# wolearyc/ramannoodle

Hardware: AMD Instinct MI355X
Metric: structures/sec (GNN polarizability eval) (higher is better)
Workload: dtype f32

## Files before the change

### ramannoodle_amd/csrc/kernels_c2_pairs.hip

```cpp
#include "fused_common.hpp"

namespace rn {

struct C2PairArgs {
  const float *node;
  float *out;
  int64_t M;
  int N, NP;
  const int *pair_a, *pair_b;
  Dims d;
  PassW<float> w;
};

namespace {
constexpr int C2P_THREADS = 256;
}

__global__ __launch_bounds__(C2P_THREADS, 2) void c2_pairs_kernel(C2PairArgs a) {
  __shared__ __attribute__((aligned(16))) float s_bias[2 * FP], s_g1[2 * FP], s_b1[2 * FP], s_g2[FP], s_b2[FP];
  const int tid = threadIdx.x, lane = tid & 63, wave = tid >> 6;
  const int l15 = lane & 15, quad = lane >> 4;
  const float sc2 = a.w.mfma_scale_c[4];
  for (int c = tid; c < 2 * FP; c += C2P_THREADS) {
    s_bias[c] = a.w.c2_bias_c[c] * sc2;
    s_g1[c] = a.w.c2_norm_1.g[c];
    s_b1[c] = a.w.c2_norm_1.b[c];
    if (c < FP) {
      s_g2[c] = a.w.c2_norm_2.g[c];
      s_b2[c] = a.w.c2_norm_2.b[c];
    }
  }
  WaveB<true> bW[4];
#pragma unroll
  for (int p = 0; p < 4; ++p) bW[p].load(a.w.c2_WT_c, 2 * FP, 32 * p, l15, quad, sc2);
  __syncthreads();

  const float inv2n = 1.0f / (float)(2 * a.d.Fe), invn = 1.0f / (float)a.d.Fe;
  const float eps_c2 = 1e-5f * sc2 * sc2;
  const int64_t ntiles = (a.M + 15) / 16, stride = (int64_t)gridDim.x * (C2P_THREADS / 64);

  f32x4 xb[4], xa[4];
  auto fetch = [&](int64_t tile) {
    int64_t row = tile * 16 + l15;
    if (row >= a.M) row = a.M - 1;
    const int64_t s = row / a.NP;
    const int p = (int)(row - s * a.NP);
    const float *nb = a.node + (s * a.N + a.pair_b[p]) * FP + 16 * quad, *na = a.node + (s * a.N + a.pair_a[p]) * FP + 16 * quad;
#pragma unroll
    for (int j = 0; j < 4; ++j) {
      xb[j] = *reinterpret_cast<const f32x4 *>(nb + 4 * j);
      xa[j] = *reinterpret_cast<const f32x4 *>(na + 4 * j);
    }
  };
  int64_t tile = (int64_t)blockIdx.x * (C2P_THREADS / 64) + wave;
  if (tile < ntiles) fetch(tile);
  for (; tile < ntiles; tile += stride) {
    float af[KS];
#pragma unroll
    for (int j = 0; j < 4; ++j) {
      const f32x4 pr = xb[j] * xa[j];
#pragma unroll
      for (int i = 0; i < 4; ++i) af[4 * j + i] = pr[i];
    }
    f16x8 ah[2], al[2];
    split_f16x8(af, ah[0], al[0]);
    split_f16x8(af + 8, ah[1], al[1]);
    if (tile + stride < ntiles) fetch(tile + stride);

    const int lq = launder(lane >> 4);
    f32x4 acc[4][2];
#pragma unroll
    for (int p = 0; p < 4; ++p) {
#pragma unroll
      for (int t = 0; t < 2; ++t) acc[p][t] = *reinterpret_cast<const f32x4 *>(s_bias + 32 * p + 16 * t + 4 * lq);
      bW[p].product_split(ah, al, acc[p]);
    }
    float q = 0.f;
#pragma unroll
    for (int p = 0; p < 4; ++p)
#pragma unroll
      for (int t = 0; t < 2; ++t)
#pragma unroll
        for (int i = 0; i < 4; ++i) q = fmaf(acc[p][t][i], acc[p][t][i], q);
    q = sum_xor32(sum_xor16(q));
    const float rstd2 = fast_rsq(q * inv2n + eps_c2);
    float gv[2][2][4], sum = 0.f;
#pragma unroll
    for (int p = 0; p < 2; ++p)
#pragma unroll
      for (int t = 0; t < 2; ++t) {
        const int c = 32 * p + 16 * t + 4 * lq;
        const Vec4<float> gf = load4<float>(s_g1 + c), bf = load4<float>(s_b1 + c);
        const Vec4<float> gc = load4<float>(s_g1 + FP + c), bc = load4<float>(s_b1 + FP + c);
#pragma unroll
        for (int i = 0; i < 4; ++i) {
          gv[p][t][i] = gate(acc[p][t][i] * rstd2 * gf.v[i] + bf.v[i], acc[p + 2][t][i] * rstd2 * gc.v[i] + bc.v[i]);
          sum += gv[p][t][i];
        }
      }
    const float mean = sum_xor32(sum_xor16(sum)) * invn;
    float qq = 0.f;
#pragma unroll
    for (int p = 0; p < 2; ++p)
#pragma unroll
      for (int t = 0; t < 2; ++t)
#pragma unroll
        for (int i = 0; i < 4; ++i) {
          const int c = 32 * p + 16 * t + 4 * lq + i;
          gv[p][t][i] = c < a.d.Fe ? gv[p][t][i] - mean : 0.f;
          qq = fmaf(gv[p][t][i], gv[p][t][i], qq);
        }
    const float rstd = fast_rsq(sum_xor32(sum_xor16(qq)) * invn + 1e-5f);
    const int64_t row = tile * 16 + l15 < a.M ? tile * 16 + l15 : a.M - 1;
    {
#pragma unroll
      for (int p = 0; p < 2; ++p)
#pragma unroll
        for (int t = 0; t < 2; ++t) {
          const int c = 32 * p + 16 * t + 4 * lq;
          const Vec4<float> g2 = load4<float>(s_g2 + c), b2 = load4<float>(s_b2 + c);
          f32x4 y;
#pragma unroll
          for (int i = 0; i < 4; ++i) y[i] = gv[p][t][i] * rstd * g2.v[i] + b2.v[i];
          *reinterpret_cast<f32x4 *>(a.out + row * FP + c) = y;
        }
    }
  }
}

void launch_c2_pairs(const float *node, float *out, int S, const Graph &g, Dims d, const PassW<float> &w, hipStream_t st) {
  const int64_t M = (int64_t)S * g.NP;
  if (M == 0) return;
  C2PairArgs a{node, out, M, g.N, g.NP, g.pair_a, g.pair_b, d, w};
  static int cus = 0;
  if (cus == 0) {
    int dev = 0;
    hipDeviceProp_t prop;
    if (hipGetDevice(&dev) == hipSuccess && hipGetDeviceProperties(&prop, dev) == hipSuccess) cus = prop.multiProcessorCount;
    if (cus <= 0) cus = 256;
  }
  const int64_t ntiles = (M + 15) / 16, per_wg = C2P_THREADS / 64;
  const int64_t grid = std::min<int64_t>((ntiles + per_wg - 1) / per_wg, (int64_t)2 * cus);
  c2_pairs_kernel<<<(unsigned)grid, C2P_THREADS, 0, st>>>(a);
}

}
```

### ramannoodle_amd/csrc/kernels_fused.hip

```cpp
#include "fused_common.hpp"

namespace rn {


#ifndef RN_NODE_REGRING
#define RN_NODE_REGRING 2
#endif
#ifndef RN_NODE_PROBE
#define RN_NODE_PROBE 0
#endif
template <bool PAD, bool F16, bool ZM = false >
__global__ __launch_bounds__(256, 4) void node_block_fused_kernel(NodeFusedArgs a) {
  extern __shared__ __attribute__((aligned(16))) unsigned char smem_raw[];
  const Graph &g = a.g;
  const NodeFusedLds L = node_fused_lds(g.nt_max_in_rows, g.nt_max_nodes);
  float *bufP = reinterpret_cast<float *>(smem_raw + L.bufP);
  float *atile = reinterpret_cast<float *>(smem_raw + L.atile);
  float *gated = reinterpret_cast<float *>(smem_raw + L.gated);
  float *nj = reinterpret_cast<float *>(smem_raw + L.nj);
  float *lnp = reinterpret_cast<float *>(smem_raw + L.lnp);
  float *s_c1g = lnp, *s_c1b = lnp + 2 * FP, *s_fg = lnp + 4 * FP, *s_fb = lnp + 5 * FP;
  int *d_edge = reinterpret_cast<int *>(smem_raw + L.ints), *d_bl = d_edge + g.nt_max_in_rows;

  const int tid = threadIdx.x, lane = tid & 63;
  const int wave = __builtin_amdgcn_readfirstlane(tid >> 6);
  const int l15 = lane & 15, quad = lane >> 4;
  const int colbase = wave * 32;
  int logical = blockIdx.x;
  if ((gridDim.x & 7) == 0) logical = (blockIdx.x & 7) * (gridDim.x >> 3) + (blockIdx.x >> 3);
  const int tile = logical % g.nt_num;
  const int sg = logical / g.nt_num, nsg = gridDim.x / g.nt_num;
  const int j0 = g.nt_begin[tile], j1 = g.nt_begin[tile + 1];
  const int di0 = g.in_ptr[j0], dcount = g.in_ptr[j1] - di0;
  const int nrounds = (dcount + NG - 1) / NG;

  for (int c = tid; c < 2 * FP; c += 256) {
    s_c1g[c] = a.w.c1_norm.g[c];
    s_c1b[c] = a.w.c1_norm.b[c];
    if (c < FP) {
      s_fg[c] = a.w.final_norm.g[c];
      s_fb[c] = a.w.final_norm.b[c];
    }
  }
  for (int i = tid; i < dcount; i += 256) {
    const int e = g.in_edge[di0 + i];
    d_edge[i] = e;
    d_bl[i] = g.edge_b[e] - j0;
  }
  WaveB<F16> bW;
  const float s1 = F16 ? (ZM ? a.w.mfma_scale_c[6] : a.w.mfma_scale[0]) : 1.0f, inv1 = F16 ? (ZM ? a.w.mfma_scale_c[7] : a.w.mfma_scale[1]) : 1.0f;
  bW.load(ZM ? a.w.c1_WeT_c : a.w.c1_WeT, 2 * FP, colbase, l15, quad, s1);

  const int grp = tid / LG, q4 = tid % LG, c0 = 4 * q4;
  const int nvalid = min(max(a.d.Fn - c0, 0), 4);
  const float inv2n = 1.0f / (float)(2 * a.d.Fn), invn = 1.0f / (float)a.d.Fn;
  __syncthreads();
  const LnParams<float> pf{load4<float>(s_c1g + c0), load4<float>(s_c1b + c0)};
  const LnParams<float> pc{load4<float>(s_c1g + FP + c0), load4<float>(s_c1b + FP + c0)};

  [[maybe_unused]] auto prefetch_round = [&](int s, int r) {
    const int row = 4 * wave + quad;
    const int i = min(r * NG + row, dcount - 1);
    const int piece = (l15 ^ row) & 15;
    dma16(a.edge + ((int64_t)s * g.E + d_edge[i]) * FP + 4 * piece, atile + wave * 256);
  };
  [[maybe_unused]] auto split_landed_tiles = [&]() {
    if constexpr (F16) {
      float *slot = atile + wave * 256 + lane * 4;
      *reinterpret_cast<float4 *>(slot) = split_slot(*reinterpret_cast<const float4 *>(slot));
    }
  };
#if RN_NODE_REGRING
  constexpr int RING = RN_NODE_REGRING;
  float4 ring[RING];
  int fs = sg, fr = 0;
  auto fetch_next = [&]() {
    float4 v = make_float4(0.f, 0.f, 0.f, 0.f);
    if (fs < a.S) {
      const int row = 4 * wave + quad;
      const int i = min(fr * NG + row, dcount - 1);
      const int piece = (l15 ^ row) & 15;
      v = *reinterpret_cast<const float4 *>(a.edge + ((int64_t)fs * g.E + d_edge[i]) * FP + 4 * piece);
      if (++fr == nrounds) {
        fr = 0;
        fs += nsg;
      }
    }
    return v;
  };
  auto publish_next = [&]() {
    float4 v = ring[0];
    if constexpr (F16) v = split_slot(v);
    *reinterpret_cast<float4 *>(atile + tid * 4) = v;
#pragma unroll
    for (int j = 0; j + 1 < RING; ++j) ring[j] = ring[j + 1];
    ring[RING - 1] = fetch_next();
  };
  if (dcount > 0) {
#pragma unroll
    for (int j = 0; j < RING; ++j) ring[j] = fetch_next();
    if (sg < a.S) publish_next();
  }
#else
  if (sg < a.S && dcount > 0) prefetch_round(sg, 0);
#endif

  for (int s = sg; s < a.S; s += nsg) {
    const int64_t nrow0 = (int64_t)s * g.N;
    for (int i = tid; i < ((RN_NODE_PROBE & 8) ? 0 : (j1 - j0) * (2 * FP / 4)); i += 256) {
      const int n = i / (2 * FP / 4), c = (i % (2 * FP / 4)) * 4;
      store4(nj + (size_t)n * 2 * FP + c, load4<float>(a.npc1 + (nrow0 + j0 + n) * (2 * FP) + c));
    }
#if !RN_NODE_REGRING
    dma_wait();
    if (s == sg) split_landed_tiles();
#endif
    __syncthreads();
    for (int r = 0; r < nrounds; ++r) {
      if (!(RN_NODE_PROBE & 1)) {
        f32x4 acc[2] = {{0.f, 0.f, 0.f, 0.f}, {0.f, 0.f, 0.f, 0.f}};
        if constexpr (F16) {
          f16x8 ah[2], al[2];
          load_split_a(atile, l15, quad, ah, al);
          bW.product_split(ah, al, acc);
        } else {
          float af[KS];
#pragma unroll
          for (int j = 0; j < 4; ++j) {
            const float4 v = *reinterpret_cast<const float4 *>(atile + l15 * FP + (((4 * quad + j) ^ l15) & 15) * 4);
            af[4 * j] = v.x; af[4 * j + 1] = v.y; af[4 * j + 2] = v.z; af[4 * j + 3] = v.w;
          }
          bW.product(af, acc);
        }
#pragma unroll
        for (int t = 0; t < 2; ++t) *reinterpret_cast<f32x4 *>(bufP + l15 * LDQ + colbase + 16 * t + 4 * quad) = acc[t];
      }
      if (!(RN_NODE_PROBE & 32))
      __syncthreads();
#if RN_NODE_REGRING
      if (r + 1 < nrounds || s + nsg < a.S) publish_next();
#else
      if (r + 1 < nrounds) prefetch_round(s, r + 1);
      else if (s + nsg < a.S) prefetch_round(s + nsg, 0);
#endif
#if RN_NODE_PRIO
      __builtin_amdgcn_s_setprio(0);
#endif
      const int i = r * NG + grp;
      if (i < dcount && !(RN_NODE_PROBE & 2)) {
        const float *njr = nj + (size_t)d_bl[i] * 2 * FP + c0;
        Vec4<float> xf = load4<float>(bufP + grp * LDQ + c0), xc = load4<float>(bufP + grp * LDQ + FP + c0);
        const Vec4<float> af = load4<float>(njr), ac = load4<float>(njr + FP);
#pragma unroll
        for (int k = 0; k < 4; ++k) {
          xf.v[k] = fmaf(xf.v[k], inv1, af.v[k]);
          xc.v[k] = fmaf(xc.v[k], inv1, ac.v[k]);
        }
        if constexpr (ZM) store4(gated + (size_t)i * LDG + c0, ln_gate_zero_mean<LG>(xf, xc, pf, pc, inv2n));
        else store4(gated + (size_t)i * LDG + c0, ln_gate<LG, PAD>(xf, xc, pf, pc, inv2n, nvalid));
      }
#if RN_NODE_PRIO
      __builtin_amdgcn_s_setprio(RN_NODE_PRIO);
#endif
#if !RN_NODE_REGRING
      dma_wait();
      if (r + 1 < nrounds || s + nsg < a.S) split_landed_tiles();
#endif
      if (!(RN_NODE_PROBE & 16) || r + 1 == nrounds)
      __syncthreads();
    }
    for (int n = grp; n < ((RN_NODE_PROBE & 4) ? 0 : j1 - j0); n += NG) {
      const int i0 = g.in_ptr[j0 + n] - di0, i1 = g.in_ptr[j0 + n + 1] - di0;
      Vec4<float> acc{{0.f, 0.f, 0.f, 0.f}};
      for (int i = i0; i < i1; ++i) {
        const Vec4<float> v = load4<float>(gated + (size_t)i * LDG + c0);
#pragma unroll
        for (int k = 0; k < 4; ++k) acc.v[k] += v.v[k];
      }
      const LnParams<float> pn{load4<float>(s_fg + c0), load4<float>(s_fb + c0)};
      const Vec4<float> ln = ln_row<LG, PAD>(acc, pn, invn, nvalid);
      const Vec4<float> old = load4<float>(a.node_in + (nrow0 + j0 + n) * FP + c0);
      Vec4<float> out;
#pragma unroll
      for (int k = 0; k < 4; ++k) out.v[k] = fast_tanh(old.v[k] + ln.v[k]);
      store4(a.node_out + (nrow0 + j0 + n) * FP + c0, out);
    }
  }
}

size_t node_fused_lds_bytes(const Graph &g) { return node_fused_lds(g.nt_max_in_rows, g.nt_max_nodes).total; }
size_t node_fused_lds_bytes(int tile_in_rows, int tile_nodes) { return node_fused_lds(tile_in_rows, tile_nodes).total; }

void launch_node_fused(const float *edge, const float *node_in, const float *npc1, float *node_out, int S,
                       const Graph &g, Dims d, const PassW<float> &w, bool f16, bool centred, hipStream_t st) {
  if (S == 0 || g.N == 0) return;
  NodeFusedArgs a{edge, node_in, npc1, node_out, S, g, d, w};
  const bool pad = d.Fn != d.FnP;
  const size_t lds = node_fused_lds_bytes(g);
  auto kern = f16 ? (centred ? (pad ? &node_block_fused_kernel<true, true, true> : &node_block_fused_kernel<false, true, true>)
                             : (pad ? &node_block_fused_kernel<true, true> : &node_block_fused_kernel<false, true>))
                  : (pad ? &node_block_fused_kernel<true, false> : &node_block_fused_kernel<false, false>);
  if (lds > 48 * 1024)
    (void)hipFuncSetAttribute(reinterpret_cast<const void *>(kern), hipFuncAttributeMaxDynamicSharedMemorySize,
                              (int)lds);
  static int cus = 0;
  if (cus == 0) {
    int dev = 0;
    hipDeviceProp_t prop;
    if (hipGetDevice(&dev) == hipSuccess && hipGetDeviceProperties(&prop, dev) == hipSuccess)
      cus = prop.multiProcessorCount;
    if (cus <= 0) cus = 256;
  }
  int per_cu = 0;
  if (hipOccupancyMaxActiveBlocksPerMultiprocessor(&per_cu, kern, 256, lds) != hipSuccess || per_cu < 1) per_cu = 1;
  per_cu = std::min(per_cu, 4);
  int nsg = per_cu * cus / g.nt_num;
  nsg = nsg < 1 ? 1 : (nsg > S ? S : nsg);
  kern<<<(unsigned)nsg * (unsigned)g.nt_num, 256, lds, st>>>(a);
}

struct ReadoutFusedArgs {
  const float *edge;
  float *pol;
  int64_t M;
  ReadoutW<float> w;
  int pol_stride;
};

template <bool F16, bool PRE = false, int NW = (F16 ? 8 : 4)>
__global__ __launch_bounds__(64 * NW, 2) void readout_fused_kernel(ReadoutFusedArgs a, int tiles_per_wave) {
  constexpr int LDW = FP + 4;
  constexpr int LDH = FP + 8;
  constexpr int kW64 = F16 ? 2 * FP * LDH * 2 : FP * LDW * 4, kW16 = F16 ? 2 * 16 * LDH * 2 : 16 * LDW * 4;
  extern __shared__ __attribute__((aligned(16))) unsigned char ro_smem[];
  unsigned char *w0_raw = ro_smem, *w3_raw = w0_raw + kW64, *w5_raw = w3_raw + kW64;
  float *slab_all = reinterpret_cast<float *>(w5_raw + kW16);
  float *s_scale0 = slab_all + NW * 16 * LDW, *s_shift0 = s_scale0 + FP, *s_b3 = s_shift0 + FP, *s_b5 = s_b3 + FP;
  const int tid = threadIdx.x, lane = tid & 63, wave = tid >> 6;
  const int l15 = lane & 15, quad = lane >> 4;
  auto put = [&](unsigned char *raw, int rows, int n, int k, float v) {
    if constexpr (F16) {
      _Float16 *h = reinterpret_cast<_Float16 *>(raw), *l = h + rows * LDH;
      const _Float16 hi = (_Float16)v;
      h[n * LDH + k] = hi;
      l[n * LDH + k] = (_Float16)(v - (float)hi);
    } else {
      reinterpret_cast<float *>(raw)[n * LDW + k] = v;
    }
  };
  const float ps0 = F16 ? a.w.mfma_scale[0] : 1.0f, inv0 = F16 ? a.w.mfma_scale[1] : 1.0f;
  const float ps3 = F16 ? a.w.mfma_scale[2] : 1.0f, inv3 = F16 ? a.w.mfma_scale[3] : 1.0f;
  const float ps5 = F16 ? a.w.mfma_scale[4] : 1.0f, inv5 = F16 ? a.w.mfma_scale[5] : 1.0f;
  for (int i = tid; i < FP * FP; i += 64 * NW) {
    const int k = i / FP, n = i % FP;
    put(w0_raw, FP, n, k, ps0 * a.w.W0T[i]);
    put(w3_raw, FP, n, k, ps3 * a.w.W3T[i]);
  }
  for (int i = tid; i < FP * 16; i += 64 * NW) {
    const int k = i / 16, n = i % 16;
    put(w5_raw, 16, n, k, ps5 * a.w.W5T[k * 32 + n]);
  }
  if (tid < FP) {
    s_scale0[tid] = a.w.scale0[tid] * inv0;
    s_shift0[tid] = a.w.shift0[tid];
    s_b3[tid] = a.w.b3[tid];
    if (tid < 16) s_b5[tid] = a.w.b5[tid];
  }
  __syncthreads();
  float *slab = slab_all + wave * 16 * LDW;
  const int64_t num_tiles = (a.M + 15) / 16;
  const int64_t first = ((int64_t)blockIdx.x * NW + wave) * tiles_per_wave;

  f16x8 ah[2], al[2];
  auto operand = [&](const float (&af)[KS]) {
    if constexpr (F16) {
      split_f16x8(af, ah[0], al[0]);
      split_f16x8(af + 8, ah[1], al[1]);
    }
  };
  auto operand_pairs = [&](const float (&af)[KS]) {
    union { float f[4]; f16x8 h; } u[4];
#pragma unroll
    for (int j = 0; j < 4; ++j)
#pragma unroll
      for (int i = 0; i < 4; ++i) u[j].f[i] = af[4 * j + i];
    ah[0] = u[0].h; al[0] = u[1].h; ah[1] = u[2].h; al[1] = u[3].h;
  };
  auto product = [&](const float (&af)[KS], const unsigned char *raw, int rows, int nt, f32x4 &acc) {
    acc = f32x4{0.f, 0.f, 0.f, 0.f};
    if constexpr (F16) {
      const _Float16 *h = reinterpret_cast<const _Float16 *>(raw) + (nt * 16 + l15) * LDH + quad * KS;
      const _Float16 *l = h + rows * LDH;
#pragma unroll
      for (int s = 0; s < 2; ++s)
        acc = mfma_split3(ah[s], al[s], *reinterpret_cast<const f16x8 *>(h + 8 * s),
                          *reinterpret_cast<const f16x8 *>(l + 8 * s), acc);
    } else {
      const float *wp = reinterpret_cast<const float *>(raw) + (nt * 16 + l15) * LDW + quad * KS;
#pragma unroll
      for (int j = 0; j < 4; ++j) {
        const float4 b = *reinterpret_cast<const float4 *>(wp + 4 * j);
        acc = __builtin_amdgcn_mfma_f32_16x16x4f32(af[4 * j], b.x, acc, 0, 0, 0);
        acc = __builtin_amdgcn_mfma_f32_16x16x4f32(af[4 * j + 1], b.y, acc, 0, 0, 0);
        acc = __builtin_amdgcn_mfma_f32_16x16x4f32(af[4 * j + 2], b.z, acc, 0, 0, 0);
        acc = __builtin_amdgcn_mfma_f32_16x16x4f32(af[4 * j + 3], b.w, acc, 0, 0, 0);
      }
    }
  };
  auto load_slab = [&](float (&af)[KS]) {
#pragma unroll
    for (int j = 0; j < 4; ++j) {
      const float4 v = *reinterpret_cast<const float4 *>(slab + l15 * LDW + quad * KS + 4 * j);
      af[4 * j] = v.x; af[4 * j + 1] = v.y; af[4 * j + 2] = v.z; af[4 * j + 3] = v.w;
    }
  };

  float nxt[KS];
  auto fetch = [&](int64_t tile) {
    int64_t row = tile * 16 + l15;
    if (row >= a.M) row = a.M - 1;
    const float *p = a.edge + row * FP + quad * KS;
#pragma unroll
    for (int j = 0; j < 4; ++j) {
      const float4 v = *reinterpret_cast<const float4 *>(p + 4 * j);
      nxt[4 * j] = v.x; nxt[4 * j + 1] = v.y; nxt[4 * j + 2] = v.z; nxt[4 * j + 3] = v.w;
    }
  };
  if (first < num_tiles) fetch(first);
  for (int it = 0; it < tiles_per_wave; ++it) {
    const int64_t tile = first + it;
    if (tile >= num_tiles) break;
    float af[KS];
#pragma unroll
    for (int k = 0; k < KS; ++k) af[k] = nxt[k];
    if (it + 1 < tiles_per_wave && tile + 1 < num_tiles) fetch(tile + 1);
    f32x4 acc;
    if constexpr (PRE) operand_pairs(af);
    else operand(af);
#pragma unroll
    for (int nt = 0; nt < 4; ++nt) {
      product(af, w0_raw, FP, nt, acc);
      const int col = nt * 16 + l15;
#pragma unroll
      for (int rr = 0; rr < 4; ++rr)
        slab[(4 * quad + rr) * LDW + col] = ssp_fast(acc[rr] * s_scale0[col] + s_shift0[col]);
    }
    load_slab(af);
    operand(af);
#pragma unroll
    for (int nt = 0; nt < 4; ++nt) {
      product(af, w3_raw, FP, nt, acc);
      const int col = nt * 16 + l15;
#pragma unroll
      for (int rr = 0; rr < 4; ++rr) slab[(4 * quad + rr) * LDW + col] = ssp_fast(fmaf(acc[rr], inv3, s_b3[col]));
    }
    load_slab(af);
    operand(af);
    product(af, w5_raw, 16, 0, acc);
#pragma unroll
    for (int rr = 0; rr < 4; ++rr) {
      const int64_t row = tile * 16 + 4 * quad + rr;
      if (row < a.M) a.pol[row * a.pol_stride + l15] = fmaf(acc[rr], inv5, s_b5[l15]);
    }
  }
}

void launch_readout_fused(const float *edge, int64_t M, const ReadoutW<float> &w, float *pol, bool f16,
                          hipStream_t st, bool pair_rows, int pol_stride) {
  if (M == 0) return;
  ReadoutFusedArgs a{edge, pol, M, w, pol_stride};
  const int64_t tiles = (M + 15) / 16;
  const int tpw = 8;
  auto launch = [&](auto kern, int nw, bool f16w) {
    constexpr int LDW = FP + 4, LDH = FP + 8;
    const size_t lds = (f16w ? (size_t)2 * (2 * FP * LDH * 2) + 2 * 16 * LDH * 2 : (size_t)2 * FP * LDW * 4 + 16 * LDW * 4) +
                       (size_t)nw * 16 * LDW * 4 + (3 * FP + 16) * 4;
    if (lds > 48 * 1024)
      (void)hipFuncSetAttribute(reinterpret_cast<const void *>(kern), hipFuncAttributeMaxDynamicSharedMemorySize, (int)lds);
    const unsigned blocks = (unsigned)((tiles + (int64_t)nw * tpw - 1) / ((int64_t)nw * tpw));
    kern<<<blocks, 64 * nw, lds, st>>>(a, tpw);
  };
  if (f16 && pair_rows) launch(&readout_fused_kernel<true, true>, 8, true);
  else if (f16) launch(&readout_fused_kernel<true>, 8, true);
  else launch(&readout_fused_kernel<false>, 4, false);
}

size_t edge_fused_lds_bytes(const Graph &g) {
  return fused_lds(g.max_tile_out_rows, g.max_tile_in_rows, g.max_tile_nodes).total;
}
size_t edge_fused_lds_bytes(int rows, int in_rows, int nodes) { return fused_lds(rows, in_rows, nodes).total; }

bool edge_fused_supported(const Graph &g, Dims d) {
  return d.FnP == 64 && d.FeP == 64 && g.E > 0 && edge_fused_lds_bytes(g) <= kFusedLdsBudget;
}

}
```

Before: 64480.

## Fold log2e into norm params, pack f32x2 math, and transpose readout MFMA outputs

In the c2 pairs kernel, the gate's exp scaling is folded into the norm-1 gamma and beta so a custom exp2-based gate with clamping can be used. Elementwise math moves to packed f32x2 FMAs, and a PAD template skips the padding mask when Fe equals FP. Per-tile 64-bit divides for pair index lookup are replaced by an incremental (s,p) stepper with byte-offset addressing. In the readout kernel, the MFMA operands are swapped so each lane writes four contiguous columns as one vector LDS store, and softplus is rewritten with exp2/log using prescaled biases. The changes trade exact exp/log paths for approximate hardware intrinsics and add more complex index bookkeeping.

```diff
diff --git a/ramannoodle_amd/csrc/kernels_c2_pairs.hip b/ramannoodle_amd/csrc/kernels_c2_pairs.hip
--- a/ramannoodle_amd/csrc/kernels_c2_pairs.hip
+++ b/ramannoodle_amd/csrc/kernels_c2_pairs.hip
@@ -6,7 +6,8 @@
   const float *node;
   float *out;
   int64_t M;
-  int N, NP;
+  int S, N, NP;
+  int step_s, step_p;
   const int *pair_a, *pair_b;
   Dims d;
   PassW<float> w;
@@ -14,17 +15,33 @@
 
 namespace {
 constexpr int C2P_THREADS = 256;
-}
-
+constexpr float kC2Clamp = 15.0f * 2.0f * kLog2e;
+
+__device__ __forceinline__ f32x2 gate_exp2(f32x2 yf, f32x2 yc) {
+  const f32x2 one2 = {1.0f, 1.0f};
+  const f32x2 e1 = {fast_exp2(yf.x), fast_exp2(yf.y)};
+  const f32x2 e2 = {fast_exp2(__builtin_amdgcn_fmed3f(yc.x, -kC2Clamp, kC2Clamp)),
+                    fast_exp2(__builtin_amdgcn_fmed3f(yc.y, -kC2Clamp, kC2Clamp))};
+  const f32x2 t = e2 + one2;
+  const f32x2 den = __builtin_elementwise_fma(e1, t, t);
+  const f32x2 rd = {fast_rcp(den.x), fast_rcp(den.y)};
+  return (e2 - one2) * rd;
+}
+__device__ __forceinline__ f32x2 lo2(const f32x4 &v) { return f32x2{v[0], v[1]}; }
+__device__ __forceinline__ f32x2 hi2(const f32x4 &v) { return f32x2{v[2], v[3]}; }
+}
+
+template <bool PAD>
 __global__ __launch_bounds__(C2P_THREADS, 2) void c2_pairs_kernel(C2PairArgs a) {
   __shared__ __attribute__((aligned(16))) float s_bias[2 * FP], s_g1[2 * FP], s_b1[2 * FP], s_g2[FP], s_b2[FP];
-  const int tid = threadIdx.x, lane = tid & 63, wave = tid >> 6;
+  const int tid = threadIdx.x, lane = tid & 63, wave = __builtin_amdgcn_readfirstlane(tid >> 6);
   const int l15 = lane & 15, quad = lane >> 4;
   const float sc2 = a.w.mfma_scale_c[4];
   for (int c = tid; c < 2 * FP; c += C2P_THREADS) {
+    const float k = c < FP ? -kLog2e : 2.0f * kLog2e;
     s_bias[c] = a.w.c2_bias_c[c] * sc2;
-    s_g1[c] = a.w.c2_norm_1.g[c];
-    s_b1[c] = a.w.c2_norm_1.b[c];
+    s_g1[c] = k * a.w.c2_norm_1.g[c];
+    s_b1[c] = k * a.w.c2_norm_1.b[c];
     if (c < FP) {
       s_g2[c] = a.w.c2_norm_2.g[c];
       s_b2[c] = a.w.c2_norm_2.b[c];
@@ -38,22 +55,55 @@
   const float inv2n = 1.0f / (float)(2 * a.d.Fe), invn = 1.0f / (float)a.d.Fe;
   const float eps_c2 = 1e-5f * sc2 * sc2;
   const int64_t ntiles = (a.M + 15) / 16, stride = (int64_t)gridDim.x * (C2P_THREADS / 64);
-
+  int64_t tile = (int64_t)blockIdx.x * (C2P_THREADS / 64) + wave;
+  if (tile >= ntiles) return;
+
+  constexpr unsigned ROWB = FP * sizeof(float);
+  const uint64_t frame_b = (uint64_t)a.N * ROWB, step_fb = (uint64_t)a.step_s * frame_b;
+  const uint64_t last_fb = (uint64_t)(a.S - 1) * frame_b;
+  int s, p;
+  {
+    const int64_t row = tile * 16 + l15;
+    s = (int)(row / a.NP);
+    p = (int)(row - (int64_t)s * a.NP);
+  }
+  uint64_t fb = (uint64_t)s * frame_b;
+
+  int ia, ib;
+  const char *frame;
+  auto step = [&]() {
+    const bool past = s >= a.S;
+    const int pp = past ? a.NP - 1 : p;
+    frame = reinterpret_cast<const char *>(a.node) + (past ? last_fb : fb);
+    ib = a.pair_b[pp];
+    ia = a.pair_a[pp];
+    p += a.step_p;
+    s += a.step_s;
+    fb += step_fb;
+    if (p >= a.NP) {
+      p -= a.NP;
+      ++s;
+      fb += frame_b;
+    }
+  };
   f32x4 xb[4], xa[4];
-  auto fetch = [&](int64_t tile) {
-    int64_t row = tile * 16 + l15;
-    if (row >= a.M) row = a.M - 1;
-    const int64_t s = row / a.NP;
-    const int p = (int)(row - s * a.NP);
-    const float *nb = a.node + (s * a.N + a.pair_b[p]) * FP + 16 * quad, *na = a.node + (s * a.N + a.pair_a[p]) * FP + 16 * quad;
+  auto fetch = [&](const char *fr, int ja, int jb, int q) {
+    const float *nb = reinterpret_cast<const float *>(fr + ((unsigned)jb * ROWB + 16 * (unsigned)sizeof(float) * q));
+    const float *na = reinterpret_cast<const float *>(fr + ((unsigned)ja * ROWB + 16 * (unsigned)sizeof(float) * q));
 #pragma unroll
     for (int j = 0; j < 4; ++j) {
       xb[j] = *reinterpret_cast<const f32x4 *>(nb + 4 * j);
       xa[j] = *reinterpret_cast<const f32x4 *>(na + 4 * j);
     }
   };
-  int64_t tile = (int64_t)blockIdx.x * (C2P_THREADS / 64) + wave;
-  if (tile < ntiles) fetch(tile);
+  {
+    step();
+    const char *fr0 = frame;
+    const int ia0 = ia, ib0 = ib;
+    step();
+    asm volatile("" ::: "memory");
+    fetch(fr0, ia0, ib0, quad);
+  }
   for (; tile < ntiles; tile += stride) {
     float af[KS];
 #pragma unroll
@@ -65,73 +115,96 @@
     f16x8 ah[2], al[2];
     split_f16x8(af, ah[0], al[0]);
     split_f16x8(af + 8, ah[1], al[1]);
-    if (tile + stride < ntiles) fetch(tile + stride);
-
-    const int lq = launder(lane >> 4);
+    const int ln = launder(lane), lq = ln >> 4;
+    if (tile + stride < ntiles) fetch(frame, ia, ib, lq);
+    step();
+
     f32x4 acc[4][2];
 #pragma unroll
-    for (int p = 0; p < 4; ++p) {
-#pragma unroll
-      for (int t = 0; t < 2; ++t) acc[p][t] = *reinterpret_cast<const f32x4 *>(s_bias + 32 * p + 16 * t + 4 * lq);
-      bW[p].product_split(ah, al, acc[p]);
-    }
-    float q = 0.f;
-#pragma unroll
-    for (int p = 0; p < 4; ++p)
+    for (int pp = 0; pp < 4; ++pp) {
+#pragma unroll
+      for (int t = 0; t < 2; ++t) acc[pp][t] = *reinterpret_cast<const f32x4 *>(s_bias + 32 * pp + 16 * t + 4 * lq);
+    }
+#pragma unroll
+    for (int pp = 0; pp < 4; ++pp) bW[pp].product_split(ah, al, acc[pp]);
+    f32x4 gf[2][2], bf[2][2], gc[2][2], bc[2][2];
+#pragma unroll
+    for (int pp = 0; pp < 2; ++pp)
+#pragma unroll
+      for (int t = 0; t < 2; ++t) {
+        const int c = 32 * pp + 16 * t + 4 * lq;
+        gf[pp][t] = *reinterpret_cast<const f32x4 *>(s_g1 + c);
+        bf[pp][t] = *reinterpret_cast<const f32x4 *>(s_b1 + c);
+        gc[pp][t] = *reinterpret_cast<const f32x4 *>(s_g1 + FP + c);
+        bc[pp][t] = *reinterpret_cast<const f32x4 *>(s_b1 + FP + c);
+      }
+    f32x2 q2[2] = {{0.f, 0.f}, {0.f, 0.f}};
+#pragma unroll
+    for (int pp = 0; pp < 4; ++pp)
+#pragma unroll
+      for (int t = 0; t < 2; ++t) {
+        q2[0] = __builtin_elementwise_fma(lo2(acc[pp][t]), lo2(acc[pp][t]), q2[0]);
+        q2[1] = __builtin_elementwise_fma(hi2(acc[pp][t]), hi2(acc[pp][t]), q2[1]);
+      }
+    const f32x2 qs = q2[0] + q2[1];
+    const float q = sum_xor32(sum_xor16(qs.x + qs.y));
+    const float rstd2 = fast_rsq(q * inv2n + eps_c2);
+    const f32x2 r2 = {rstd2, rstd2};
+    f32x2 gv[2][2][2], sum2 = {0.f, 0.f};
+#pragma unroll
+    for (int pp = 0; pp < 2; ++pp)
+#pragma unroll
+      for (int t = 0; t < 2; ++t) {
+        gv[pp][t][0] = gate_exp2(__builtin_elementwise_fma(lo2(acc[pp][t]) * r2, lo2(gf[pp][t]), lo2(bf[pp][t])),
+                                 __builtin_elementwise_fma(lo2(acc[pp + 2][t]) * r2, lo2(gc[pp][t]), lo2(bc[pp][t])));
+        gv[pp][t][1] = gate_exp2(__builtin_elementwise_fma(hi2(acc[pp][t]) * r2, hi2(gf[pp][t]), hi2(bf[pp][t])),
+                                 __builtin_elementwise_fma(hi2(acc[pp + 2][t]) * r2, hi2(gc[pp][t]), hi2(bc[pp][t])));
+        sum2 += gv[pp][t][0] + gv[pp][t][1];
+      }
+    const float mean = sum_xor32(sum_xor16(sum2.x + sum2.y)) * invn;
+    const f32x2 m2 = {mean, mean};
+    f32x2 qq2 = {0.f, 0.f};
+#pragma unroll
+    for (int pp = 0; pp < 2; ++pp)
 #pragma unroll
       for (int t = 0; t < 2; ++t)
 #pragma unroll
-        for (int i = 0; i < 4; ++i) q = fmaf(acc[p][t][i], acc[p][t][i], q);
-    q = sum_xor32(sum_xor16(q));
-    const float rstd2 = fast_rsq(q * inv2n + eps_c2);
-    float gv[2][2][4], sum = 0.f;
-#pragma unroll
-    for (int p = 0; p < 2; ++p)
-#pragma unroll
-      for (int t = 0; t < 2; ++t) {
-        const int c = 32 * p + 16 * t + 4 * lq;
-        const Vec4<float> gf = load4<float>(s_g1 + c), bf = load4<float>(s_b1 + c);
-        const Vec4<float> gc = load4<float>(s_g1 + FP + c), bc = load4<float>(s_b1 + FP + c);
-#pragma unroll
-        for (int i = 0; i < 4; ++i) {
-          gv[p][t][i] = gate(acc[p][t][i] * rstd2 * gf.v[i] + bf.v[i], acc[p + 2][t][i] * rstd2 * gc.v[i] + bc.v[i]);
-          sum += gv[p][t][i];
+        for (int h = 0; h < 2; ++h) {
+          gv[pp][t][h] -= m2;
+          if constexpr (PAD) {
+            const int c = 32 * pp + 16 * t + 4 * lq + 2 * h;
+            if (c >= a.d.Fe) gv[pp][t][h].x = 0.f;
+            if (c + 1 >= a.d.Fe) gv[pp][t][h].y = 0.f;
+          }
+          qq2 = __builtin_elementwise_fma(gv[pp][t][h], gv[pp][t][h], qq2);
         }
-      }
-    const float mean = sum_xor32(sum_xor16(sum)) * invn;
-    float qq = 0.f;
-#pragma unroll
-    for (int p = 0; p < 2; ++p)
-#pragma unroll
-      for (int t = 0; t < 2; ++t)
-#pragma unroll
-        for (int i = 0; i < 4; ++i) {
-          const int c = 32 * p + 16 * t + 4 * lq + i;
-          gv[p][t][i] = c < a.d.Fe ? gv[p][t][i] - mean : 0.f;
-          qq = fmaf(gv[p][t][i], gv[p][t][i], qq);
-        }
-    const float rstd = fast_rsq(sum_xor32(sum_xor16(qq)) * invn + 1e-5f);
-    const int64_t row = tile * 16 + l15 < a.M ? tile * 16 + l15 : a.M - 1;
-    {
-#pragma unroll
-      for (int p = 0; p < 2; ++p)
-#pragma unroll
-        for (int t = 0; t < 2; ++t) {
-          const int c = 32 * p + 16 * t + 4 * lq;
-          const Vec4<float> g2 = load4<float>(s_g2 + c), b2 = load4<float>(s_b2 + c);
-          f32x4 y;
-#pragma unroll
-          for (int i = 0; i < 4; ++i) y[i] = gv[p][t][i] * rstd * g2.v[i] + b2.v[i];
-          *reinterpret_cast<f32x4 *>(a.out + row * FP + c) = y;
-        }
-    }
+    f32x4 g2[2][2], b2[2][2];
+#pragma unroll
+    for (int pp = 0; pp < 2; ++pp)
+#pragma unroll
+      for (int t = 0; t < 2; ++t) {
+        const int c = 32 * pp + 16 * t + 4 * lq;
+        g2[pp][t] = *reinterpret_cast<const f32x4 *>(s_g2 + c);
+        b2[pp][t] = *reinterpret_cast<const f32x4 *>(s_b2 + c);
+      }
+    const float rstd = fast_rsq(sum_xor32(sum_xor16(qq2.x + qq2.y)) * invn + 1e-5f);
+    const f32x2 rs2 = {rstd, rstd};
+    const unsigned last = (unsigned)std::min<int64_t>(a.M - tile * 16, 16) - 1u, lrow = (unsigned)(ln & 15);
+    char *orow = reinterpret_cast<char *>(a.out) + tile * (16 * ROWB) + ((lrow < last ? lrow : last) * ROWB + 4 * (unsigned)sizeof(float) * lq);
+#pragma unroll
+    for (int pp = 0; pp < 2; ++pp)
+#pragma unroll
+      for (int t = 0; t < 2; ++t) {
+        const f32x2 y0 = __builtin_elementwise_fma(gv[pp][t][0] * rs2, lo2(g2[pp][t]), lo2(b2[pp][t]));
+        const f32x2 y1 = __builtin_elementwise_fma(gv[pp][t][1] * rs2, hi2(g2[pp][t]), hi2(b2[pp][t]));
+        *reinterpret_cast<f32x4 *>(orow + (32 * pp + 16 * t) * sizeof(float)) = f32x4{y0.x, y0.y, y1.x, y1.y};
+      }
   }
 }
 
 void launch_c2_pairs(const float *node, float *out, int S, const Graph &g, Dims d, const PassW<float> &w, hipStream_t st) {
   const int64_t M = (int64_t)S * g.NP;
   if (M == 0) return;
-  C2PairArgs a{node, out, M, g.N, g.NP, g.pair_a, g.pair_b, d, w};
   static int cus = 0;
   if (cus == 0) {
     int dev = 0;
@@ -141,7 +214,10 @@
   }
   const int64_t ntiles = (M + 15) / 16, per_wg = C2P_THREADS / 64;
   const int64_t grid = std::min<int64_t>((ntiles + per_wg - 1) / per_wg, (int64_t)2 * cus);
-  c2_pairs_kernel<<<(unsigned)grid, C2P_THREADS, 0, st>>>(a);
-}
-
-}
+  const int64_t step_rows = grid * per_wg * 16;
+  C2PairArgs a{node, out, M, S, g.N, g.NP, (int)(step_rows / g.NP), (int)(step_rows % g.NP), g.pair_a, g.pair_b, d, w};
+  if (d.Fe < FP) c2_pairs_kernel<true><<<(unsigned)grid, C2P_THREADS, 0, st>>>(a);
+  else c2_pairs_kernel<false><<<(unsigned)grid, C2P_THREADS, 0, st>>>(a);
+}
+
+}
diff --git a/ramannoodle_amd/csrc/kernels_fused.hip b/ramannoodle_amd/csrc/kernels_fused.hip
--- a/ramannoodle_amd/csrc/kernels_fused.hip
+++ b/ramannoodle_amd/csrc/kernels_fused.hip
@@ -227,6 +227,13 @@
   int pol_stride;
 };
 
+namespace {
+__device__ __forceinline__ float ssp_exp2(float y) {
+  const float t = __builtin_amdgcn_exp2f(-fabsf(y));
+  return fmaf(0.6931471805599453f, fmaxf(y, 0.0f) + __builtin_amdgcn_logf(1.0f + t), -0.6931471805599453f);
+}
+}
+
 template <bool F16, bool PRE = false, int NW = (F16 ? 8 : 4)>
 __global__ __launch_bounds__(64 * NW, 2) void readout_fused_kernel(ReadoutFusedArgs a, int tiles_per_wave) {
   constexpr int LDW = FP + 4;
@@ -251,6 +258,7 @@
   const float ps0 = F16 ? a.w.mfma_scale[0] : 1.0f, inv0 = F16 ? a.w.mfma_scale[1] : 1.0f;
   const float ps3 = F16 ? a.w.mfma_scale[2] : 1.0f, inv3 = F16 ? a.w.mfma_scale[3] : 1.0f;
   const float ps5 = F16 ? a.w.mfma_scale[4] : 1.0f, inv5 = F16 ? a.w.mfma_scale[5] : 1.0f;
+  const float inv3l = inv3 * kLog2e;
   for (int i = tid; i < FP * FP; i += 64 * NW) {
     const int k = i / FP, n = i % FP;
     put(w0_raw, FP, n, k, ps0 * a.w.W0T[i]);
@@ -261,9 +269,9 @@
     put(w5_raw, 16, n, k, ps5 * a.w.W5T[k * 32 + n]);
   }
   if (tid < FP) {
-    s_scale0[tid] = a.w.scale0[tid] * inv0;
-    s_shift0[tid] = a.w.shift0[tid];
-    s_b3[tid] = a.w.b3[tid];
+    s_scale0[tid] = a.w.scale0[tid] * inv0 * kLog2e;
+    s_shift0[tid] = a.w.shift0[tid] * kLog2e;
+    s_b3[tid] = a.w.b3[tid] * kLog2e;
     if (tid < 16) s_b5[tid] = a.w.b5[tid];
   }
   __syncthreads();
@@ -307,11 +315,33 @@
       }
     }
   };
+  auto product_t = [&](const float (&af)[KS], const unsigned char *raw, int rows, int nt, f32x4 &acc) {
+    acc = f32x4{0.f, 0.f, 0.f, 0.f};
+    if constexpr (F16) {
+      const _Float16 *h = reinterpret_cast<const _Float16 *>(raw) + (nt * 16 + l15) * LDH + quad * KS;
+      const _Float16 *l = h + rows * LDH;
+#pragma unroll
+      for (int s = 0; s < 2; ++s)
+        acc = mfma_split3(*reinterpret_cast<const f16x8 *>(h + 8 * s), *reinterpret_cast<const f16x8 *>(l + 8 * s), ah[s],
+                          al[s], acc);
+    } else {
+      const float *wp = reinterpret_cast<const float *>(raw) + (nt * 16 + l15) * LDW + quad * KS;
+#pragma unroll
+      for (int j = 0; j < 4; ++j) {
+        const float4 b = *reinterpret_cast<const float4 *>(wp + 4 * j);
+        acc = __builtin_amdgcn_mfma_f32_16x16x4f32(b.x, af[4 * j], acc, 0, 0, 0);
+        acc = __builtin_amdgcn_mfma_f32_16x16x4f32(b.y, af[4 * j + 1], acc, 0, 0, 0);
+        acc = __builtin_amdgcn_mfma_f32_16x16x4f32(b.z, af[4 * j + 2], acc, 0, 0, 0);
+        acc = __builtin_amdgcn_mfma_f32_16x16x4f32(b.w, af[4 * j + 3], acc, 0, 0, 0);
+      }
+    }
+  };
   auto load_slab = [&](float (&af)[KS]) {
+    const float *rd = slab + launder(l15 * LDW + quad * KS);
 #pragma unroll
     for (int j = 0; j < 4; ++j) {
-      const float4 v = *reinterpret_cast<const float4 *>(slab + l15 * LDW + quad * KS + 4 * j);
-      af[4 * j] = v.x; af[4 * j + 1] = v.y; af[4 * j + 2] = v.z; af[4 * j + 3] = v.w;
+      const f32x4 v = *reinterpret_cast<const f32x4 *>(rd + 4 * j);
+      af[4 * j] = v[0]; af[4 * j + 1] = v[1]; af[4 * j + 2] = v[2]; af[4 * j + 3] = v[3];
     }
   };
 
@@ -339,20 +369,25 @@
     else operand(af);
 #pragma unroll
     for (int nt = 0; nt < 4; ++nt) {
-      product(af, w0_raw, FP, nt, acc);
-      const int col = nt * 16 + l15;
-#pragma unroll
-      for (int rr = 0; rr < 4; ++rr)
-        slab[(4 * quad + rr) * LDW + col] = ssp_fast(acc[rr] * s_scale0[col] + s_shift0[col]);
+      product_t(af, w0_raw, FP, nt, acc);
+      const int col = nt * 16 + 4 * quad;
+      const f32x4 sc = *reinterpret_cast<const f32x4 *>(s_scale0 + col), sh = *reinterpret_cast<const f32x4 *>(s_shift0 + col);
+      f32x4 hid;
+#pragma unroll
+      for (int i = 0; i < 4; ++i) hid[i] = ssp_exp2(fmaf(acc[i], sc[i], sh[i]));
+      *reinterpret_cast<f32x4 *>(slab + l15 * LDW + col) = hid;
     }
     load_slab(af);
     operand(af);
 #pragma unroll
     for (int nt = 0; nt < 4; ++nt) {
-      product(af, w3_raw, FP, nt, acc);
-      const int col = nt * 16 + l15;
-#pragma unroll
-      for (int rr = 0; rr < 4; ++rr) slab[(4 * quad + rr) * LDW + col] = ssp_fast(fmaf(acc[rr], inv3, s_b3[col]));
+      product_t(af, w3_raw, FP, nt, acc);
+      const int col = nt * 16 + 4 * quad;
+      const f32x4 b3 = *reinterpret_cast<const f32x4 *>(s_b3 + col);
+      f32x4 hid;
+#pragma unroll
+      for (int i = 0; i < 4; ++i) hid[i] = ssp_exp2(fmaf(acc[i], inv3l, b3[i]));
+      *reinterpret_cast<f32x4 *>(slab + l15 * LDW + col) = hid;
     }
     load_slab(af);
     operand(af);
```

New measurement: 64550 (median of 2 runs). Within noise of the previous version (+0.1%).
